# Rikorose/DeepFilterNet

Hardware: AMD Instinct MI355X
Metric: 48 kHz audio frames/sec (hop=480), DeepFilterNet3 enhance() (higher is better)
Workload: dtype f32 (storage and accumulation; GRU projections / recurrences, the fused DF-encoder convolutions and the pointwise halves of the ERB separable convolutions as fp16-split MFMAs: x = hi + lo in f16, hi*hi + hi*lo + lo*hi on v_mfma_f32_16x16x32_f16, ~2^-21 relative; see exact_fp32_ms_per_step); 1 GPU; DeepFilterNet3 (recalled shipped shape, conv_ch=64) enhance(pad=True), batch=256 clips x 10 s @48 kHz per GPU, 1002 STFT frames per clip; batch_per_gpu=256, global_batch=256, parallelism=clips sharded over 1 GPU(s); no collective, inputs_resident_in_hbm=True

## Files before the change

### deepfilternet_amd/csrc/dfx_nn_kernels.h

```cpp
#pragma once

#include "dfx_common.h"

#include <type_traits>

#define DFX_ACT_NONE 0
#define DFX_ACT_RELU 1
#define DFX_ACT_TANH 2
#define DFX_ACT_SIGMOID 3

static __device__ __forceinline__ float dfx_sigmoid(float x) { return 1.f / (1.f + expf(-x)); }
static __device__ __forceinline__ float dfx_act(float v, int act) {
    if (act == DFX_ACT_RELU) return fmaxf(v, 0.f);
    if (act == DFX_ACT_TANH) return tanhf(v);
    if (act == DFX_ACT_SIGMOID) return dfx_sigmoid(v);
    return v;
}

template <int I, int N, typename F>
static __device__ __forceinline__ void dfx_static_for(F &&f) {
    if constexpr (I < N) {
        f(std::integral_constant<int, I>{});
        dfx_static_for<I + 1, N>(f);
    }
// ... 267 lines not shown
                                         fmaxf(acc[nt][2] + biasr[nt].z, 0.f), fmaxf(acc[nt][3] + biasr[nt].w, 0.f));
        }
    }
}

static __device__ __forceinline__ void dfx_c0_patch(const float *__restrict__ feat, int64_t b, int64_t t, int f, bool valid,
                                                    int64_t T, int Fin, int L, int q, float (&bv)[5]) {
#pragma unroll
    for (int ks = 0; ks < 5; ++ks) {
        const int k = 4 * ks + q, tap = k >> 1, ch = k & 1, kt = tap / 3, kf = tap - 3 * kt;
        const int64_t tau = t - 2 + kt, tin = tau + L;
        const int fin = f - 1 + kf;
        float v = 0.f;
        if (valid && k < 18 && tau >= 0 && tin < T && fin >= 0 && fin < Fin) v = feat[((b * T + tin) * Fin + fin) * 2 + ch];
        bv[ks] = v;
    }
}

template <int C>
static __device__ __forceinline__ void dfx_c0_tile(const float (&areg0)[C / 16][5], const float4 (&bias0)[C / 16],
                                                   const float (&bv)[5], bool keep, float (&dst)[C / 4]) {
    constexpr int NT = C / 16;
    f32x4 acc[NT];
#pragma unroll
    for (int nt = 0; nt < NT; ++nt) acc[nt] = f32x4{0.f, 0.f, 0.f, 0.f};
#pragma unroll
    for (int ks = 0; ks < 5; ++ks)
#pragma unroll
        for (int nt = 0; nt < NT; ++nt) acc[nt] = __builtin_amdgcn_mfma_f32_16x16x4f32(areg0[nt][ks], bv[ks], acc[nt], 0, 0, 0);
#pragma unroll
    for (int nt = 0; nt < NT; ++nt) {
        dst[4 * nt + 0] = keep ? fmaxf(acc[nt][0] + bias0[nt].x, 0.f) : 0.f;
        dst[4 * nt + 1] = keep ? fmaxf(acc[nt][1] + bias0[nt].y, 0.f) : 0.f;
        dst[4 * nt + 2] = keep ? fmaxf(acc[nt][2] + bias0[nt].z, 0.f) : 0.f;
        dst[4 * nt + 3] = keep ? fmaxf(acc[nt][3] + bias0[nt].w, 0.f) : 0.f;
    }
}

struct DfxC01Args {
    const float *feat;
    const float *weff0;
    const float *bias0;
    const float *dw;
    const float *wt;
    const float *bias;
    float *out;
    int64_t B, T;
    int Fin, Fout, stride, L;
    int64_t t_begin;
    int64_t t_end;
};

template <int C>
__global__ void __launch_bounds__(DFX_PW_THREADS) dfx_k_df_conv01(DfxC01Args A) {
    constexpr int CPL = C / 4, NT = C / 16;
    __shared__ float4 dws[3 * C / 4];
    const int tid = threadIdx.x, lane = tid & 63, wave = tid >> 6, q = lane >> 4, jl = lane & 15;
    for (int i = tid; i < 3 * C / 4; i += DFX_PW_THREADS) dws[i] = reinterpret_cast<const float4 *>(A.dw)[i];
    float areg0[NT][5];
#pragma unroll
    for (int nt = 0; nt < NT; ++nt)
#pragma unroll
        for (int ks = 0; ks < 5; ++ks) areg0[nt][ks] = A.weff0[(4 * ks + q) * C + 16 * nt + jl];
    float areg[NT][CPL];
#pragma unroll
    for (int nt = 0; nt < NT; ++nt)
#pragma unroll
        for (int ks = 0; ks < CPL; ++ks) areg[nt][ks] = A.wt[(16 * (ks >> 2) + 4 * q + (ks & 3)) * C + 16 * nt + jl];
    float4 bias0[NT], biasr[NT];
#pragma unroll
    for (int nt = 0; nt < NT; ++nt) {
        bias0[nt] = reinterpret_cast<const float4 *>(A.bias0)[4 * nt + q];
        biasr[nt] = reinterpret_cast<const float4 *>(A.bias)[4 * nt + q];
    }
    __syncthreads();
    const int64_t Tn = A.t_end - A.t_begin;
    const int64_t total = A.B * Tn * A.Fout;
    const int64_t ntiles = (total + 15) / 16;
    for (int64_t tile = (int64_t)blockIdx.x * 4 + wave; tile < ntiles; tile += (int64_t)gridDim.x * 4) {
        const int64_t lpos = tile * 16 + jl;
        const bool valid = lpos < total;
        const int64_t rl = lpos / A.Fout;
        const int fo = (int)(lpos - rl * A.Fout);
        const int64_t b = rl / Tn, t = A.t_begin + (rl - b * Tn);
        const int64_t pos = (b * A.T + t) * A.Fout + fo;
        float u[CPL];
#pragma unroll
        for (int i = 0; i < CPL; ++i) u[i] = 0.f;
#pragma unroll
        for (int j = 0; j < 3; ++j) {
            const int fi = fo * A.stride + j - 1;
            const bool ok = valid && fi >= 0 && fi < A.Fin;
            float bv[5], c0v[CPL];
            dfx_c0_patch(A.feat, b, t, fi, ok, A.T, A.Fin, A.L, q, bv);
            dfx_c0_tile<C>(areg0, bias0, bv, ok, c0v);
#pragma unroll
            for (int nt = 0; nt < NT; ++nt) {
                const float4 w = dws[j * (C / 4) + 4 * nt + q];
                u[4 * nt + 0] += w.x * c0v[4 * nt + 0];
                u[4 * nt + 1] += w.y * c0v[4 * nt + 1];
                u[4 * nt + 2] += w.z * c0v[4 * nt + 2];
                u[4 * nt + 3] += w.w * c0v[4 * nt + 3];
            }
        }
        f32x4 acc[NT];
#pragma unroll
        for (int nt = 0; nt < NT; ++nt) acc[nt] = f32x4{0.f, 0.f, 0.f, 0.f};
#pragma unroll
        for (int ks = 0; ks < CPL; ++ks)
#pragma unroll
            for (int nt = 0; nt < NT; ++nt) acc[nt] = __builtin_amdgcn_mfma_f32_16x16x4f32(areg[nt][ks], u[ks], acc[nt], 0, 0, 0);
        if (valid) {
            float4 *op = reinterpret_cast<float4 *>(A.out + pos * C + 4 * q);
#pragma unroll
            for (int nt = 0; nt < NT; ++nt)
                op[4 * nt] = make_float4(fmaxf(acc[nt][0] + biasr[nt].x, 0.f), fmaxf(acc[nt][1] + biasr[nt].y, 0.f),
                                         fmaxf(acc[nt][2] + biasr[nt].z, 0.f), fmaxf(acc[nt][3] + biasr[nt].w, 0.f));
        }
    }
}

static __device__ __forceinline__ void dfx_c0_patch_load(const float *__restrict__ feat, int64_t b, int64_t t, int f, bool valid,
                                                         int64_t T, int Fin, int L, int q, float2 (&raw)[4], int64_t Ts = 0) {
    if (Ts <= 0) Ts = T;
#pragma unroll
    for (int i = 0; i < 4; ++i) {
        const int tap = 4 * q + i, kt = tap / 3, kf = tap - 3 * kt;
        const int64_t tau = t - 2 + kt, tin = tau + L;
        const int fin = f - 1 + kf;
        float2 v = make_float2(0.f, 0.f);
        if (valid && tap < 9 && tau >= 0 && tin < T && fin >= 0 && fin < Fin)
            v = *reinterpret_cast<const float2 *>(feat + ((b * Ts + tin) * Fin + fin) * 2);
        raw[i] = v;
    }
}

typedef unsigned dfx_words4 __attribute__((vector_size(16)));
struct DfxPatchPs {
    dfx_words4 h, l;
};
static __device__ __forceinline__ void dfx_c0_patch_ps(const DfxPatchPs &pk, dfx_h8 &ph, dfx_h8 &pl) {
    ph = __builtin_bit_cast(dfx_h8, pk.h);
    pl = __builtin_bit_cast(dfx_h8, pk.l);
}
static __device__ __forceinline__ void dfx_put_tap(float2 (&p)[4], int i, bool in, float2 v) { p[i] = make_float2(in ? v.x : 0.f, in ? v.y : 0.f); }
static __device__ __forceinline__ void dfx_put_tap(DfxPatchPs &p, int i, bool in, uint2 v) { p.h[i] = in ? v.x : 0u, p.l[i] = in ? v.y : 0u; }
static __device__ __forceinline__ void dfx_copy_patch(float2 (&d)[4], const float2 (&s)[4]) {
#pragma unroll
    for (int i = 0; i < 4; ++i) d[i] = s[i];
}
static __device__ __forceinline__ void dfx_copy_patch(DfxPatchPs &d, const DfxPatchPs &s) { d = s; }

template <int C>
static __device__ __forceinline__ void dfx_c0_tile_h3p(const dfx_h8 (&w0h)[C / 16], const dfx_h8 (&w0l)[C / 16],
                                                       const float4 (&bias0)[C / 16], float unscale0, const dfx_h8 ph, const dfx_h8 pl,
                                                       bool keep, float (&dst)[C / 4]) {
    constexpr int NT = C / 16;
    f32x4 acc[NT];
#pragma unroll
    for (int nt = 0; nt < NT; ++nt) acc[nt] = dfx_mfma_16x16x32_f16(w0l[nt], ph, f32x4{0.f, 0.f, 0.f, 0.f});
#pragma unroll
    for (int nt = 0; nt < NT; ++nt) acc[nt] = dfx_mfma_16x16x32_f16(w0h[nt], pl, acc[nt]);
#pragma unroll
    for (int nt = 0; nt < NT; ++nt) acc[nt] = dfx_mfma_16x16x32_f16(w0h[nt], ph, acc[nt]);
#pragma unroll
    for (int nt = 0; nt < NT; ++nt) {
        dst[4 * nt + 0] = keep ? fmaxf(acc[nt][0] * unscale0 + bias0[nt].x, 0.f) : 0.f;
        dst[4 * nt + 1] = keep ? fmaxf(acc[nt][1] * unscale0 + bias0[nt].y, 0.f) : 0.f;
        dst[4 * nt + 2] = keep ? fmaxf(acc[nt][2] * unscale0 + bias0[nt].z, 0.f) : 0.f;
        dst[4 * nt + 3] = keep ? fmaxf(acc[nt][3] * unscale0 + bias0[nt].w, 0.f) : 0.f;
    }
}
template <int C>
static __device__ __forceinline__ void dfx_c0_tile_h3(const dfx_h8 (&w0h)[C / 16], const dfx_h8 (&w0l)[C / 16],
                                                      const float4 (&bias0)[C / 16], float unscale0, const float2 (&raw)[4],
                                                      bool keep, float (&dst)[C / 4], float &amax) {
    float x[8];
#pragma unroll
    for (int i = 0; i < 4; ++i) x[2 * i] = raw[i].x, x[2 * i + 1] = raw[i].y;
    dfx_h8 ph, pl;
    dfx_split8_g(x, ph, pl, amax);
    dfx_c0_tile_h3p<C>(w0h, w0l, bias0, unscale0, ph, pl, keep, dst);
}
template <int C>
static __device__ __forceinline__ void dfx_c0_tile_h3(const dfx_h8 (&w0h)[C / 16], const dfx_h8 (&w0l)[C / 16],
                                                      const float4 (&bias0)[C / 16], float unscale0, const DfxPatchPs &raw,
                                                      bool keep, float (&dst)[C / 4], float &) {
    dfx_h8 ph, pl;
    dfx_c0_patch_ps(raw, ph, pl);
    dfx_c0_tile_h3p<C>(w0h, w0l, bias0, unscale0, ph, pl, keep, dst);
}

struct DfxC01hArgs {
    const float *feat;
    const dfx_h8 *w0f;
    const float *bias0;
    const float *dw;
    const dfx_h8 *wpf;
    const float *bias;
    float *out;
    int64_t B, T;
    int Fin, Fout, stride, L;
    float unscale0, unscale;
    int64_t t_begin;
    int64_t t_end;
    unsigned int *err;
    int64_t feat_T = 0;
};

template <int C>
#ifndef DFX_C01_MINB
#define DFX_C01_MINB 3
#endif
#ifndef DFX_C01_PIN
#define DFX_C01_PIN 0
#endif
#ifndef DFX_C01_EPI_BATCH
#define DFX_C01_EPI_BATCH 2
#endif
__global__ void __launch_bounds__(DFX_PW_THREADS, DFX_C01_MINB) dfx_k_df_conv01_h3(DfxC01hArgs A) {
    constexpr int CPL = C / 4, NT = C / 16, KC = C >= 32 ? C / 32 : 1, C4 = C / 4;
    static_assert(C % 32 == 0, "one k-chunk is 32 channels");
    __shared__ float4 dws[3 * C4];
    __shared__ float4 b0s[C4], b1s[C4];
    __shared__ dfx_h8 wps[NT * KC * 2 * 64];
    const int tid = threadIdx.x, lane = tid & 63, wave = tid >> 6, q = lane >> 4, jl = lane & 15;
    for (int i = tid; i < 3 * C4; i += DFX_PW_THREADS) dws[i] = reinterpret_cast<const float4 *>(A.dw)[i];
    for (int i = tid; i < C4; i += DFX_PW_THREADS) {
        b0s[i] = reinterpret_cast<const float4 *>(A.bias0)[i];
        b1s[i] = reinterpret_cast<const float4 *>(A.bias)[i];
    }
    for (int i = tid; i < NT * KC * 2 * 64; i += DFX_PW_THREADS) wps[i] = A.wpf[i];
    dfx_h8 w0h[NT], w0l[NT];
#pragma unroll
    for (int nt = 0; nt < NT; ++nt) {
        w0h[nt] = A.w0f[(nt * 2 + 0) * 64 + lane];
        w0l[nt] = A.w0f[(nt * 2 + 1) * 64 + lane];
    }
    __syncthreads();
    const unsigned Tn = (unsigned)(A.t_end - A.t_begin);
    const unsigned NF = (unsigned)A.B * Tn;
    const int TPF = (A.Fout + 15) >> 4;
    const unsigned nwaves = gridDim.x * 4;
    const int T32 = (int)A.T, Fin = A.Fin, Lk = A.L;
    int tdt[4], tdf[4];
    bool tok[4];
#pragma unroll
    for (int i = 0; i < 4; ++i) {
        const int tap = 4 * q + i, kt = tap / 3;
        tok[i] = tap < 9;
        tdt[i] = kt - 2 + Lk;
        tdf[i] = tap - 3 * kt - 1;
    }
    float2 raw[3][4];
    bool okj[3];
    const unsigned wid = (unsigned)blockIdx.x * 4 + (unsigned)dfx_wave_uniform(wave);
    const unsigned step_fr = nwaves / (unsigned)TPF;
    const int step_ft = (int)(nwaves - step_fr * (unsigned)TPF);
    unsigned nfr = wid / (unsigned)TPF;
    int nft = (int)(wid - nfr * (unsigned)TPF), nb = 0, nt_ = 0;
    bool nlive = nfr < NF;
    auto settle = [&]() {
        if (nlive) {
            nb = (int)(nfr / Tn);
            nt_ = (int)A.t_begin + (int)(nfr - (unsigned)nb * Tn);
        }
    };
    settle();
    auto issue = [&](int j) {
        const int fo = nft * 16 + jl;
        const int fi = fo * A.stride + j - 1;
        okj[j] = nlive && fo < A.Fout && fi >= 0 && fi < Fin;
        const float2 *clip = reinterpret_cast<const float2 *>(A.feat) + (int64_t)nb * (A.feat_T > 0 ? A.feat_T : (int64_t)T32) * Fin;
#pragma unroll
        for (int i = 0; i < 4; ++i) {
            const int tin = nt_ + tdt[i], fin = fi + tdf[i];
            float2 v = make_float2(0.f, 0.f);
            if (okj[j] && tok[i] && tin - Lk >= 0 && tin < T32 && fin >= 0 && fin < Fin) v = clip[tin * Fin + fin];
            raw[j][i] = v;
        }
    };
    float amax = 0.f;
#pragma unroll
    for (int j = 0; j < 3; ++j) issue(j);
    while (nlive) {
        const int fo_c = nft * 16 + jl;
        const bool valid = fo_c < A.Fout;
        const int64_t pos = ((int64_t)nb * T32 + nt_) * A.Fout + fo_c;
        nft += step_ft;
        nfr += step_fr;
        if (nft >= TPF) nft -= TPF, ++nfr;
        nlive = nfr < NF;
        settle();
        float u[CPL];
#pragma unroll
        for (int i = 0; i < CPL; ++i) u[i] = 0.f;
#pragma unroll
        for (int j = 0; j < 3; ++j) {
            float x[8];
#pragma unroll
            for (int i = 0; i < 4; ++i) x[2 * i] = raw[j][i].x, x[2 * i + 1] = raw[j][i].y;
            const bool keep = okj[j];
            dfx_h8 ph, pl;
            dfx_split8_g(x, ph, pl, amax);
            issue(j);
            f32x4 acc[NT];
#pragma unroll
            for (int nt = 0; nt < NT; ++nt) acc[nt] = dfx_mfma_16x16x32_f16(w0l[nt], ph, f32x4{0.f, 0.f, 0.f, 0.f});
#pragma unroll
            for (int nt = 0; nt < NT; ++nt) acc[nt] = dfx_mfma_16x16x32_f16(w0h[nt], pl, acc[nt]);
#pragma unroll
            for (int nt = 0; nt < NT; ++nt) acc[nt] = dfx_mfma_16x16x32_f16(w0h[nt], ph, acc[nt]);
#if DFX_C01_PIN
#pragma unroll
            for (int n0 = 0; n0 < NT; n0 += DFX_C01_EPI_BATCH) {
                float4 bz[DFX_C01_EPI_BATCH], w[DFX_C01_EPI_BATCH];
#pragma unroll
                for (int d = 0; d < DFX_C01_EPI_BATCH; ++d) {
                    bz[d] = b0s[4 * (n0 + d) + q], w[d] = dws[j * C4 + 4 * (n0 + d) + q];
                    DFX_OPAQUE(bz[d].x);
                    DFX_OPAQUE(bz[d].y);
                    DFX_OPAQUE(bz[d].z);
                    DFX_OPAQUE(bz[d].w);
                    DFX_OPAQUE(w[d].x);
// ... 160 lines not shown
                    const int tin = t + (tinfo[i] & 0xff) - 64, fin = fi + ((tinfo[i] >> 8) & 0xff) - 1;
                    float2 v = make_float2(0.f, 0.f);
                    if (ok && (tinfo[i] >> 16) && tin - Lk >= 0 && tin < T32 && fin >= 0 && fin < Fin) v = feat2[cbase + (unsigned)(tin * Fin + fin)];
                    dst[i] = v;
                }
            }
        };
        auto c0_tile = [&](auto jc, auto addc, auto nextc, int fo, Patch &rw, float (&u)[CPL], bool refill) {
            constexpr int j = decltype(jc)::value;
            constexpr bool ADD = decltype(addc)::value, NEXT = decltype(nextc)::value;
            const int fi = fo * A.stride + j - 1;
            const bool keep = live && fi >= 0 && fi < Fin;
            dfx_h8 ph, pl;
            if constexpr (PS) {
                dfx_c0_patch_ps(rw, ph, pl);
            } else {
                float x[8];
#pragma unroll
                for (int i = 0; i < 4; ++i) x[2 * i] = rw[i].x, x[2 * i + 1] = rw[i].y;
                dfx_split8_g(x, ph, pl, amax);
            }
            if (refill) issue_to(rw, j, fo + 1);
            int z0 = 0;
            DFX_OPAQUE(z0);
            dfx_h8 w0h[NT], w0l[NT];
#pragma unroll
            for (int nt = 0; nt < NT; ++nt) {
                w0h[nt] = w0s[(nt * 2 + 0) * 64 + lane + z0];
                w0l[nt] = w0s[(nt * 2 + 1) * 64 + lane + z0];
            }
            f32x4 acc[NT];
#pragma unroll
            for (int nt = 0; nt < NT; ++nt) acc[nt] = dfx_mfma_16x16x32_f16(w0l[nt], ph, f32x4{0.f, 0.f, 0.f, 0.f});
#pragma unroll
            for (int nt = 0; nt < NT; ++nt) acc[nt] = dfx_mfma_16x16x32_f16(w0h[nt], pl, acc[nt]);
#pragma unroll
            for (int nt = 0; nt < NT; ++nt) acc[nt] = dfx_mfma_16x16x32_f16(w0h[nt], ph, acc[nt]);
            auto epilogue = [&](auto allc) {
                constexpr bool ALL = decltype(allc)::value;
#pragma unroll
                for (int nt = 0; nt < NT; ++nt) {
                    const float4 bz = b0s[4 * nt + q];
                    const float v0 = ALL || keep ? fmaxf(acc[nt][0] * A.unscale0 + bz.x, 0.f) : 0.f, v1 = ALL || keep ? fmaxf(acc[nt][1] * A.unscale0 + bz.y, 0.f) : 0.f;
                    const float v2 = ALL || keep ? fmaxf(acc[nt][2] * A.unscale0 + bz.z, 0.f) : 0.f, v3 = ALL || keep ? fmaxf(acc[nt][3] * A.unscale0 + bz.w, 0.f) : 0.f;
                    if constexpr (ADD) {
                        const float4 w = dws[j * C4 + 4 * nt + q];
                        u[4 * nt + 0] += w.x * v0;
                        u[4 * nt + 1] += w.y * v1;
                        u[4 * nt + 2] += w.z * v2;
                        u[4 * nt + 3] += w.w * v3;
                    }
                    if constexpr (NEXT) {
                        const float4 wn = dws[4 * nt + q];
                        uns[nt * DFX_PW_THREADS + tid] = make_float4(0.f + wn.x * v0, 0.f + wn.y * v1, 0.f + wn.z * v2, 0.f + wn.w * v3);
                    }
                }
            };
            if constexpr (PS) {
                if (fi >= 0 && fi < Fin) epilogue(std::true_type{});
                else epilogue(std::false_type{});
            } else {
                epilogue(std::false_type{});
            }
        };
        using I0 = std::integral_constant<int, 0>;
        using I1 = std::integral_constant<int, 1>;
        using I2 = std::integral_constant<int, 2>;
        f32x4 accg = f32x4{0.f, 0.f, 0.f, 0.f};
        float ev[8];
        int ci = fo0 * KC;
        {
            float none[CPL];
            issue_to(raw[0], 0, fo0);
            c0_tile(I0{}, std::false_type{}, std::true_type{}, fo0, raw[0], none, false);
            issue_to(raw[0], 1, fo0);
            issue_to(raw[1], 2, fo0);
        }
        for (int fo = fo0; fo < fo1; ++fo) {
            float u[CPL];
#pragma unroll
            for (int nt = 0; nt < NT; ++nt) {
                const float4 c = uns[nt * DFX_PW_THREADS + tid];
                u[4 * nt + 0] = c.x, u[4 * nt + 1] = c.y, u[4 * nt + 2] = c.z, u[4 * nt + 3] = c.w;
            }
            c0_tile(I1{}, std::true_type{}, std::false_type{}, fo, raw[0], u, true);
            c0_tile(I2{}, std::true_type{}, std::true_type{}, fo, raw[1], u, true);
            dfx_h8 uh[KC], ul[KC];
#pragma unroll
            for (int kc = 0; kc < KC; ++kc) dfx_split8_g(u + 8 * kc, uh[kc], ul[kc], amax);
            int zoff = 0;
            DFX_OPAQUE(zoff);
            const dfx_h8 *wpl_ = wps + lane + zoff;
#pragma unroll
            for (int kc = 0; kc < KC; ++kc, ++ci) {
                int lz = lane;
                DFX_OPAQUE(lz);
                const dfx_h8 *wfl_ = A.wfc + lz;
                const dfx_h8 fh = wfl_[((size_t)ci * 2 + 0) * 64], fl = wfl_[((size_t)ci * 2 + 1) * 64];
                float c1v[8];
#pragma unroll
                for (int h = 0; h < 2; ++h) {
                    const int nt = 2 * kc + h;
                    f32x4 aa = f32x4{0.f, 0.f, 0.f, 0.f}, ab = aa, ac = aa;
#pragma unroll
                    for (int k2 = 0; k2 < KC; ++k2) {
                        const dfx_h8 wh = wpl_[((nt * KC + k2) * 2 + 0) * 64], wl = wpl_[((nt * KC + k2) * 2 + 1) * 64];
                        aa = dfx_mfma_16x16x32_f16(wl, uh[k2], aa);
                        ab = dfx_mfma_16x16x32_f16(wh, ul[k2], ab);
                        ac = dfx_mfma_16x16x32_f16(wh, uh[k2], ac);
                    }
                    const float4 bz = b1s[4 * nt + q];
                    c1v[4 * h + 0] = fmaxf(((aa[0] + ab[0]) + ac[0]) * A.unscale + bz.x, 0.f);
                    c1v[4 * h + 1] = fmaxf(((aa[1] + ab[1]) + ac[1]) * A.unscale + bz.y, 0.f);
                    c1v[4 * h + 2] = fmaxf(((aa[2] + ab[2]) + ac[2]) * A.unscale + bz.z, 0.f);
                    c1v[4 * h + 3] = fmaxf(((aa[3] + ab[3]) + ac[3]) * A.unscale + bz.w, 0.f);
                }
                dfx_h8 ch, cl;
                dfx_split8_g(c1v, ch, cl, amax);
                accg = dfx_mfma_16x16x32_f16(fl, ch, accg);
                accg = dfx_mfma_16x16x32_f16(fh, cl, accg);
                accg = dfx_mfma_16x16x32_f16(fh, ch, accg);
                if ((ci + 1) % A.cpg == 0) {
                    const int g = ci / A.cpg;
                    float4 e = make_float4(0.f, 0.f, 0.f, 0.f);
                    if (live) e = *reinterpret_cast<const float4 *>(A.e3 + (row * (unsigned)emb + (unsigned)(16 * g + 4 * q)));
                    const float4 v = make_float4(fmaxf(accg[0] * A.unscale_fc, 0.f) + e.x, fmaxf(accg[1] * A.unscale_fc, 0.f) + e.y,
                                                 fmaxf(accg[2] * A.unscale_fc, 0.f) + e.z, fmaxf(accg[3] * A.unscale_fc, 0.f) + e.w);
                    if (A.emb_in && live) *reinterpret_cast<float4 *>(A.emb_in + (row * (unsigned)emb + (unsigned)(16 * g + 4 * q))) = v;
                    accg = f32x4{0.f, 0.f, 0.f, 0.f};
                    if (g & 1) {
                        ev[4] = v.x, ev[5] = v.y, ev[6] = v.z, ev[7] = v.w;
                        const int jg = g >> 1;
                        const dfx_h8 *wil_ = A.win + lane + zoff;
                        const dfx_h8 ih = wil_[((size_t)jg * 2 + 0) * 64], il = wil_[((size_t)jg * 2 + 1) * 64];
                        dfx_h8 eh, el;
                        dfx_split8_g(ev, eh, el, amax);
                        f32x4 o = dfx_mfma_16x16x32_f16(il, eh, f32x4{0.f, 0.f, 0.f, 0.f});
                        o = dfx_mfma_16x16x32_f16(ih, el, o);
                        o = dfx_mfma_16x16x32_f16(ih, eh, o);
                        if (live)
                            *reinterpret_cast<float4 *>(A.xa + (row * (unsigned)(emb / 2) + (unsigned)(16 * jg + 4 * q))) =
                                make_float4(fmaxf(o[0] * A.unscale_in, 0.f), fmaxf(o[1] * A.unscale_in, 0.f), fmaxf(o[2] * A.unscale_in, 0.f),
                                            fmaxf(o[3] * A.unscale_in, 0.f));
                    } else {
                        ev[0] = v.x, ev[1] = v.y, ev[2] = v.z, ev[3] = v.w;
                    }
                }
            }
        }
    }
    if (amax >= DFX_H3_LIMIT && A.err) dfx_raise(A.err + 1);
}

struct DfxCphArgs {
    const float *feat;
    const dfx_h8 *w0f;
    const float *bias0;
    const dfx_h8 *wf;
    const float *bias;
    float *out;
    int64_t B, T;
    int Fd, NO, nfb, nseg, tseg, L;
    float unscale0, unscale;
    int64_t t_begin, t_zero, t_end;
    unsigned int *err;
    int64_t feat_T = 0;
    const int *t_zero_rows = nullptr;
    const uint2 *feat_ps = nullptr;
};

template <int C, int KT, bool PS = false>
__global__ void __launch_bounds__(256, 1) dfx_k_df_convp_h3(DfxCphArgs A) {
    using Patch = std::conditional_t<PS, DfxPatchPs, float2[4]>;
    using Elem = std::conditional_t<PS, uint2, float2>;
    constexpr int CPL = C / 4, NT = C / 16, KC = C >= 32 ? C / 32 : 1;
    static_assert(C % 32 == 0, "one k-chunk is 32 channels");
    const int tid = threadIdx.x, lane = tid & 63, wave = tid >> 6, q = lane >> 4, jl = lane & 15;
    float4 bias0[NT];
#pragma unroll
    for (int nt = 0; nt < NT; ++nt) bias0[nt] = reinterpret_cast<const float4 *>(A.bias0)[4 * nt + q];
    dfx_h8 w0h[NT], w0l[NT], wh[KT][KC], wl[KT][KC];
#pragma unroll
    for (int nt = 0; nt < NT; ++nt) {
        w0h[nt] = A.w0f[(nt * 2 + 0) * 64 + lane];
        w0l[nt] = A.w0f[(nt * 2 + 1) * 64 + lane];
    }
#pragma unroll
    for (int k = 0; k < KT; ++k)
#pragma unroll
        for (int kc = 0; kc < KC; ++kc) {
            wh[k][kc] = A.wf[((k * KC + kc) * 2 + 0) * 64 + lane];
            wl[k][kc] = A.wf[((k * KC + kc) * 2 + 1) * 64 + lane];
            DFX_PIN_AGPR(wh[k][kc]);
            DFX_PIN_AGPR(wl[k][kc]);
        }
    float biasr[4];
#pragma unroll
    for (int r = 0; r < 4; ++r) biasr[r] = A.bias[4 * q + r];
    const int64_t nruns = A.B * A.nfb * A.nseg;
    float amax = 0.f;
    const int Fd = A.Fd, T32 = (int)A.T, Lk = A.L;
    const int fT = (int)(A.feat_T > 0 ? A.feat_T : A.T);
    int toff[4], tdt[4], tdf[4];
#pragma unroll
    for (int i = 0; i < 4; ++i) {
        const int tap = 4 * q + i, kt = tap / 3;
        tdt[i] = tap < 9 ? kt - 2 + Lk : (1 << 20);
        tdf[i] = tap - 3 * kt - 1;
        toff[i] = (kt - 2 + Lk) * Fd + tdf[i];
    }
    const Elem *feat2;
    if constexpr (PS) feat2 = A.feat_ps;
    else feat2 = reinterpret_cast<const float2 *>(A.feat);
    for (int64_t run = (int64_t)blockIdx.x * 4 + dfx_wave_uniform(wave); run < nruns; run += (int64_t)gridDim.x * 4) {
        const int seg = (int)(run % A.nseg);
        const int64_t rest = run / A.nseg;
        const int fb = (int)(rest % A.nfb);
        const int64_t b = rest / A.nfb;
        const int f = fb * 16 + jl;
        const bool fvalid = f < Fd;
        const int64_t t0 = A.t_begin + (int64_t)seg * A.tseg;
        const int64_t t1 = (t0 + A.tseg < A.t_end) ? t0 + A.tseg : A.t_end;
        const unsigned cbase = (unsigned)b * (unsigned)fT * (unsigned)Fd;
        const int64_t tz = A.t_zero_rows ? (int64_t)A.t_zero_rows[b] : A.t_zero;
        auto patch = [&](int t, bool ok, Patch &rw) {
            const unsigned pbase = cbase + (unsigned)(t * Fd + f);
#pragma unroll
            for (int i = 0; i < 4; ++i) {
                const int tin = t + tdt[i], fin = f + tdf[i];
                const bool in = ok && tin - Lk >= 0 && tin < T32 && fin >= 0 && fin < Fd;
                dfx_put_tap(rw, i, in, feat2[in ? pbase + (unsigned)toff[i] : cbase]);
            }
        };
        dfx_h8 xh[KT][KC], xl[KT][KC];
        Patch raw;
        auto make_frame = [&](dfx_h8 (&dh)[KC], dfx_h8 (&dl)[KC], int64_t tau, const Patch &rw) {
            float c0v[CPL];
            dfx_c0_tile_h3<C>(w0h, w0l, bias0, A.unscale0, rw, fvalid && tau >= tz, c0v, amax);
#pragma unroll
            for (int kc = 0; kc < KC; ++kc) dfx_split8_g(c0v + 8 * kc, dh[kc], dl[kc], amax);
        };
        dfx_static_for<1, KT>([&](auto sc) {
            constexpr int sl = decltype(sc)::value;
            const int64_t tau = t0 - KT + sl;
            patch((int)tau, fvalid && tau >= 0, raw);
            make_frame(xh[sl], xl[sl], tau, raw);
        });
        patch((int)t0, fvalid, raw);
        for (int64_t tb = t0; tb < t1; tb += KT) {
            dfx_static_for<0, KT>([&](auto pc) {
                constexpr int ph = decltype(pc)::value;
                const int64_t t = tb + ph;
                if (t < t1) {
                    Patch cur;
                    dfx_copy_patch(cur, raw);
                    patch((int)t + 1, fvalid && t + 1 < t1, raw);
                    make_frame(xh[ph], xl[ph], t, cur);
                    f32x4 aa = f32x4{0.f, 0.f, 0.f, 0.f}, ab = aa, ac = aa;
                    dfx_static_for<0, KT>([&](auto kcn) {
                        constexpr int k = decltype(kcn)::value;
                        constexpr int sl = (ph + 1 + k) % KT;
#pragma unroll
                        for (int kc = 0; kc < KC; ++kc) {
                            const dfx_h8 whk = wh[k][kc], wlk = wl[k][kc];
                            aa = dfx_mfma_16x16x32_f16(wlk, xh[sl][kc], aa);
                            ab = dfx_mfma_16x16x32_f16(whk, xl[sl][kc], ab);
                            ac = dfx_mfma_16x16x32_f16(whk, xh[sl][kc], ac);
                        }
                    });
                    f32x4 acc;
#pragma unroll
                    for (int r = 0; r < 4; ++r) acc[r] = (aa[r] + ab[r]) + ac[r];
                    if (fvalid) {
                        float *op = A.out + ((b * (A.NO / 2) * A.T + t) * A.Fd + f) * 2;
#pragma unroll
                        for (int h = 0; h < 2; ++h)
                            if (4 * q + 2 * h < A.NO)
                                *reinterpret_cast<float2 *>(op + (int64_t)(2 * q + h) * A.T * A.Fd * 2) =
                                    make_float2(fmaxf(acc[2 * h] * A.unscale + biasr[2 * h], 0.f),
                                                fmaxf(acc[2 * h + 1] * A.unscale + biasr[2 * h + 1], 0.f));
                    }
                }
            });
        }
    }
    if (amax >= DFX_H3_LIMIT && A.err) dfx_raise(A.err + 1);
}

template <int C, int KT, bool REBUILD>
__global__ void __launch_bounds__(256, REBUILD ? 1 : 2) dfx_k_df_convp_step(DfxCphArgs A, f32x4 *pend, int slot_new, const unsigned char *par = nullptr,
                                                             const int *cnt = nullptr) {
    constexpr int CPL = C / 4, NT = C / 16, KC = C / 32, NS = KT - 1;
    static_assert(C % 32 == 0 && KT >= 2, "one k-chunk is 32 channels; kt = 1 has no history");
    const int tid = threadIdx.x, lane = tid & 63, wave = tid >> 6, q = lane >> 4, jl = lane & 15;
    dfx_h8 w0h[NT], w0l[NT];
    float4 bias0[NT];
#pragma unroll
    for (int nt = 0; nt < NT; ++nt) {
        w0h[nt] = A.w0f[(nt * 2 + 0) * 64 + lane];
        w0l[nt] = A.w0f[(nt * 2 + 1) * 64 + lane];
        bias0[nt] = reinterpret_cast<const float4 *>(A.bias0)[4 * nt + q];
    }
    float biasr[4];
#pragma unroll
    for (int r = 0; r < 4; ++r) biasr[r] = A.bias[4 * q + r];
    const int64_t nruns = A.B * A.nfb;
    const int64_t t = A.T - 1;
    float amax = 0.f;
    for (int64_t run = (int64_t)blockIdx.x * 4 + wave; run < nruns; run += (int64_t)gridDim.x * 4) {
        const int fb = (int)(run % A.nfb);
        const int64_t b = run / A.nfb;
        const int f = fb * 16 + jl;
        const bool fvalid = f < A.Fd;
        const int64_t tz = A.t_zero_rows ? (int64_t)A.t_zero_rows[dfx_wave_uniform((int)b)] : A.t_zero;
        const int half_in = par ? (int)(par[b] & 1) : 0, half_out = par ? half_in ^ 1 : 0, halves = par ? 2 : 1;
        const int slot0 = cnt ? cnt[b] % NS : slot_new;
        auto slot_ptr = [&](int j, int half) { return pend + ((((size_t)b * halves + half) * NS + (slot0 + j) % NS) * A.nfb + fb) * 64 + lane; };
        f32x4 sa[KT], sb[KT], sc[KT];
#pragma unroll
        for (int o = 0; o < KT; ++o) sa[o] = sb[o] = f32x4{0.f, 0.f, 0.f, 0.f}, sc[o] = f32x4{0.f, 0.f, 0.f, 0.f};
        if (!REBUILD) {
#pragma unroll
            for (int o = 0; o < NS; ++o) sc[o] = *slot_ptr(o, half_in);
        }
        dfx_static_for<(REBUILD ? 0 : KT - 1), KT>([&](auto dc) {
            constexpr int d = decltype(dc)::value;
            const int64_t tau = t - (KT - 1) + d;
            float2 raw[4];
            dfx_c0_patch_load(A.feat, b, tau, f, fvalid && tau >= 0, A.T, A.Fd, A.L, q, raw, A.feat_T);
            float c0v[CPL];
            dfx_c0_tile_h3<C>(w0h, w0l, bias0, A.unscale0, raw, fvalid && tau >= tz, c0v, amax);
            dfx_h8 xh[KC], xl[KC];
#pragma unroll
            for (int kc = 0; kc < KC; ++kc) dfx_split8_g(c0v + 8 * kc, xh[kc], xl[kc], amax);
            int zoff = 0;
            DFX_OPAQUE(zoff);
            const dfx_h8 *wfl = A.wf + lane + zoff;
#pragma unroll
            for (int kc = 0; kc < KC; ++kc) {
                dfx_h8 wl[KT], wh[KT];
                dfx_static_for<0, d + 1>([&](auto kcn) {
                    constexpr int k = decltype(kcn)::value;
                    wl[k] = wfl[((k * KC + kc) * 2 + 1) * 64], wh[k] = wfl[((k * KC + kc) * 2 + 0) * 64];
                });
                dfx_static_for<0, d + 1>([&](auto kcn) { constexpr int k = decltype(kcn)::value; sa[d - k] = dfx_mfma_16x16x32_f16(wl[k], xh[kc], sa[d - k]); });
                dfx_static_for<0, d + 1>([&](auto kcn) { constexpr int k = decltype(kcn)::value; sb[d - k] = dfx_mfma_16x16x32_f16(wh[k], xl[kc], sb[d - k]); });
                dfx_static_for<0, d + 1>([&](auto kcn) { constexpr int k = decltype(kcn)::value; sc[d - k] = dfx_mfma_16x16x32_f16(wh[k], xh[kc], sc[d - k]); });
            }
        });
        f32x4 sum[KT];
#pragma unroll
        for (int o = 0; o < KT; ++o)
#pragma unroll
            for (int r = 0; r < 4; ++r) sum[o][r] = (sa[o][r] + sb[o][r]) + sc[o][r];
#pragma unroll
        for (int o = 1; o < KT; ++o) *slot_ptr(o, half_out) = sum[o];
        if (fvalid) {
            float *op = A.out + ((b * (A.NO / 2) * A.T + t) * A.Fd + f) * 2;
#pragma unroll
            for (int h = 0; h < 2; ++h)
                if (4 * q + 2 * h < A.NO)
                    *reinterpret_cast<float2 *>(op + (int64_t)(2 * q + h) * A.T * A.Fd * 2) =
                        make_float2(fmaxf(sum[0][2 * h] * A.unscale + biasr[2 * h], 0.f), fmaxf(sum[0][2 * h + 1] * A.unscale + biasr[2 * h + 1], 0.f));
        }
    }
    if (amax >= DFX_H3_LIMIT && A.err) dfx_raise(A.err + 1);
}

#define DFX_CH_NF 2
template <int C, int MODE, typename Epi>
static __device__ __forceinline__ void dfx_chain_stage(const float *in, int Fin, int Fout, int stride, int npos,
                                                       const float4 *dws, const float (&areg)[C / 16][C / 4],
                                                       const float4 (&biasr)[C / 16], int lane, Epi &&epi) {
    constexpr int CPL = C / 4, NT = C / 16, V4 = CPL / 4, LD = C + 4;
    const int q = lane >> 4, jl = lane & 15;
    for (int p0 = 0; p0 < npos; p0 += 16) {
        const int p = p0 + jl;
        const bool valid = p < npos;
        const int fr = p / Fout, fo = p - fr * Fout;
        float u[CPL];
#pragma unroll
        for (int i = 0; i < CPL; ++i) u[i] = 0.f;
#pragma unroll
        for (int j = 0; j < 3; ++j) {
            int fi;
            bool ok;
            if (MODE == DFX_PW_MODE_DW3) {
                fi = fo * stride + j - 1;
                ok = fi >= 0 && fi < Fin;
            } else {
                const int num = fo + 1 - j;
                fi = num >> 1;
                ok = num >= 0 && (num & 1) == 0 && fi < Fin;
            }
            if (valid && ok) {
                const float4 *xp = reinterpret_cast<const float4 *>(in + (fr * Fin + fi) * LD + CPL * q);
#pragma unroll
                for (int v = 0; v < V4; ++v) {
                    const float4 xv = xp[v];
                    const float4 w = dws[j * (C / 4) + V4 * q + v];
                    u[4 * v + 0] += w.x * xv.x;
                    u[4 * v + 1] += w.y * xv.y;
                    u[4 * v + 2] += w.z * xv.z;
                    u[4 * v + 3] += w.w * xv.w;
                }
            }
        }
        f32x4 acc[NT];
#pragma unroll
        for (int nt = 0; nt < NT; ++nt) acc[nt] = f32x4{0.f, 0.f, 0.f, 0.f};
#pragma unroll
        for (int ks = 0; ks < CPL; ++ks)
#pragma unroll
            for (int nt = 0; nt < NT; ++nt) acc[nt] = __builtin_amdgcn_mfma_f32_16x16x4f32(areg[nt][ks], u[ks], acc[nt], 0, 0, 0);
#pragma unroll
        for (int nt = 0; nt < NT; ++nt)
            epi(p, valid, nt,
                make_float4(fmaxf(acc[nt][0] + biasr[nt].x, 0.f), fmaxf(acc[nt][1] + biasr[nt].y, 0.f),
                            fmaxf(acc[nt][2] + biasr[nt].z, 0.f), fmaxf(acc[nt][3] + biasr[nt].w, 0.f)));
    }
}

template <int C>
static __device__ __forceinline__ void dfx_chain_load_w(const float *wt, const float *bias, int lane, float (&areg)[C / 16][C / 4],
                                                        float4 (&biasr)[C / 16]) {
    constexpr int CPL = C / 4, NT = C / 16;
    const int q = lane >> 4, jl = lane & 15;
#pragma unroll
    for (int nt = 0; nt < NT; ++nt) {
#pragma unroll
        for (int ks = 0; ks < CPL; ++ks) areg[nt][ks] = wt[(CPL * q + ks) * C + 16 * nt + jl];
        biasr[nt] = reinterpret_cast<const float4 *>(bias)[4 * nt + q];
    }
}

template <int C>
static __device__ __forceinline__ void dfx_chain_load_w_h3(const dfx_h8 *frags, const float *bias, int lane, dfx_h8 (&ahi)[C / 16][C / 32],
                                                           dfx_h8 (&alo)[C / 16][C / 32], float4 (&biasr)[C / 16]) {
// ... 3258 lines not shown
```

Before: 24.28 million frames/s.

## Software-pipeline DF conv kernel: prefetch two frames ahead, delay stores, interleave MFMA/VALU

```diff
diff --git a/deepfilternet_amd/csrc/dfx_nn_kernels.h b/deepfilternet_amd/csrc/dfx_nn_kernels.h
--- a/deepfilternet_amd/csrc/dfx_nn_kernels.h
+++ b/deepfilternet_amd/csrc/dfx_nn_kernels.h
@@ -443,24 +443,37 @@
 static __device__ __forceinline__ void dfx_copy_patch(DfxPatchPs &d, const DfxPatchPs &s) { d = s; }
 
 template <int C>
+static __device__ __forceinline__ void dfx_c0_tile_h3_products(const dfx_h8 (&w0h)[C / 16], const dfx_h8 (&w0l)[C / 16], const dfx_h8 ph,
+                                                               const dfx_h8 pl, f32x4 (&acc)[C / 16]) {
+    constexpr int NT = C / 16;
+#pragma unroll
+    for (int nt = 0; nt < NT; ++nt) acc[nt] = dfx_mfma_16x16x32_f16(w0l[nt], ph, f32x4{0.f, 0.f, 0.f, 0.f});
+#pragma unroll
+    for (int nt = 0; nt < NT; ++nt) acc[nt] = dfx_mfma_16x16x32_f16(w0h[nt], pl, acc[nt]);
+#pragma unroll
+    for (int nt = 0; nt < NT; ++nt) acc[nt] = dfx_mfma_16x16x32_f16(w0h[nt], ph, acc[nt]);
+}
+template <int C>
+static __device__ __forceinline__ void dfx_c0_tile_h3_epilogue(const f32x4 (&acc)[C / 16], const float4 (&bias0)[C / 16], float unscale0, bool keep,
+                                                               float (&dst)[C / 4]) {
+    constexpr int NT = C / 16;
+#pragma unroll
+    for (int nt = 0; nt < NT; ++nt) {
+        const float v0 = fmaxf(acc[nt][0] * unscale0 + bias0[nt].x, 0.f), v1 = fmaxf(acc[nt][1] * unscale0 + bias0[nt].y, 0.f);
+        const float v2 = fmaxf(acc[nt][2] * unscale0 + bias0[nt].z, 0.f), v3 = fmaxf(acc[nt][3] * unscale0 + bias0[nt].w, 0.f);
+        dst[4 * nt + 0] = keep ? v0 : 0.f;
+        dst[4 * nt + 1] = keep ? v1 : 0.f;
+        dst[4 * nt + 2] = keep ? v2 : 0.f;
+        dst[4 * nt + 3] = keep ? v3 : 0.f;
+    }
+}
+template <int C>
 static __device__ __forceinline__ void dfx_c0_tile_h3p(const dfx_h8 (&w0h)[C / 16], const dfx_h8 (&w0l)[C / 16],
                                                        const float4 (&bias0)[C / 16], float unscale0, const dfx_h8 ph, const dfx_h8 pl,
                                                        bool keep, float (&dst)[C / 4]) {
-    constexpr int NT = C / 16;
-    f32x4 acc[NT];
-#pragma unroll
-    for (int nt = 0; nt < NT; ++nt) acc[nt] = dfx_mfma_16x16x32_f16(w0l[nt], ph, f32x4{0.f, 0.f, 0.f, 0.f});
-#pragma unroll
-    for (int nt = 0; nt < NT; ++nt) acc[nt] = dfx_mfma_16x16x32_f16(w0h[nt], pl, acc[nt]);
-#pragma unroll
-    for (int nt = 0; nt < NT; ++nt) acc[nt] = dfx_mfma_16x16x32_f16(w0h[nt], ph, acc[nt]);
-#pragma unroll
-    for (int nt = 0; nt < NT; ++nt) {
-        dst[4 * nt + 0] = keep ? fmaxf(acc[nt][0] * unscale0 + bias0[nt].x, 0.f) : 0.f;
-        dst[4 * nt + 1] = keep ? fmaxf(acc[nt][1] * unscale0 + bias0[nt].y, 0.f) : 0.f;
-        dst[4 * nt + 2] = keep ? fmaxf(acc[nt][2] * unscale0 + bias0[nt].z, 0.f) : 0.f;
-        dst[4 * nt + 3] = keep ? fmaxf(acc[nt][3] * unscale0 + bias0[nt].w, 0.f) : 0.f;
-    }
+    f32x4 acc[C / 16];
+    dfx_c0_tile_h3_products<C>(w0h, w0l, ph, pl, acc);
+    dfx_c0_tile_h3_epilogue<C>(acc, bias0, unscale0, keep, dst);
 }
 template <int C>
 static __device__ __forceinline__ void dfx_c0_tile_h3(const dfx_h8 (&w0h)[C / 16], const dfx_h8 (&w0l)[C / 16],
@@ -927,6 +940,40 @@
     if (amax >= DFX_H3_LIMIT && A.err) dfx_raise(A.err + 1);
 }
 
+#ifndef DFX_CPH_ABLATE
+#define DFX_CPH_ABLATE 0
+#endif
+#ifndef DFX_CPH_TRACE
+#define DFX_CPH_TRACE 0
+#endif
+#ifndef DFX_CPH_PARENT_LOOP
+#define DFX_CPH_PARENT_LOOP 0
+#endif
+#ifndef DFX_CPH_VALU_C0
+#define DFX_CPH_VALU_C0 4
+#endif
+#ifndef DFX_CPH_VALU_TAPS
+#define DFX_CPH_VALU_TAPS 5
+#endif
+template <int N, int V>
+static __device__ __forceinline__ void dfx_sched_mfma_valu() {
+#pragma unroll
+    for (int i = 0; i < N; ++i) {
+        DFX_SCHED_GROUP(0x008, 1);
+        DFX_SCHED_GROUP(0x002, V);
+    }
+}
+#if DFX_CPH_TRACE
+#define DFX_CPH_TICK(i)                                                               \
+    do {                                                                                \
+        unsigned long long now_;                                                        \
+        asm volatile("s_memtime %0\n\ts_waitcnt lgkmcnt(0)" : "=s"(now_)::"memory");    \
+        tk[i] += now_ - tlast;                                                          \
+        tlast = now_;                                                                   \
+    } while (0)
+#else
+#define DFX_CPH_TICK(i) do { } while (0)
+#endif
 struct DfxCphArgs {
     const float *feat;
     const dfx_h8 *w0f;
@@ -942,7 +989,29 @@
     int64_t feat_T = 0;
     const int *t_zero_rows = nullptr;
     const uint2 *feat_ps = nullptr;
+#if DFX_CPH_TRACE
+    unsigned long long *trace = nullptr;
+#endif
 };
+static __device__ __forceinline__ void dfx_patch_ready(float2 (&p)[4]) {
+#pragma unroll
+    for (int i = 0; i < 4; ++i) {
+        DFX_OPAQUE(p[i].x);
+        DFX_OPAQUE(p[i].y);
+    }
+}
+static __device__ __forceinline__ void dfx_patch_ready(DfxPatchPs &p) {
+    DFX_OPAQUE(p.h);
+    DFX_OPAQUE(p.l);
+}
+template <typename E>
+static __device__ __forceinline__ void dfx_loads_ready(E (&ld)[4]) {
+#pragma unroll
+    for (int i = 0; i < 4; ++i) {
+        DFX_OPAQUE(ld[i].x);
+        DFX_OPAQUE(ld[i].y);
+    }
+}
 
 template <int C, int KT, bool PS = false>
 __global__ void __launch_bounds__(256, 1) dfx_k_df_convp_h3(DfxCphArgs A) {
@@ -974,6 +1043,9 @@
     for (int r = 0; r < 4; ++r) biasr[r] = A.bias[4 * q + r];
     const int64_t nruns = A.B * A.nfb * A.nseg;
     float amax = 0.f;
+#if DFX_CPH_TRACE
+    unsigned long long tk[4] = {0, 0, 0, 0}, tlast, nframes = 0;
+#endif
     const int Fd = A.Fd, T32 = (int)A.T, Lk = A.L;
     const int fT = (int)(A.feat_T > 0 ? A.feat_T : A.T);
     int toff[4], tdt[4], tdf[4];
@@ -1004,14 +1076,50 @@
             for (int i = 0; i < 4; ++i) {
                 const int tin = t + tdt[i], fin = f + tdf[i];
                 const bool in = ok && tin - Lk >= 0 && tin < T32 && fin >= 0 && fin < Fd;
-                dfx_put_tap(rw, i, in, feat2[in ? pbase + (unsigned)toff[i] : cbase]);
+                if constexpr (DFX_CPH_ABLATE & 2) dfx_put_tap(rw, i, false, Elem{});
+                else dfx_put_tap(rw, i, in, feat2[in ? pbase + (unsigned)toff[i] : cbase]);
+            }
+        };
+        auto patch_in = [&](int t, bool ok, int i) {
+            return ok & (t + tdt[i] - Lk >= 0) & (t + tdt[i] < T32) & (f + tdf[i] >= 0) & (f + tdf[i] < Fd);
+        };
+        auto patch_load = [&](int t, bool ok, Elem (&ld)[4]) {
+            const unsigned pbase = cbase + (unsigned)(t * Fd + f);
+#pragma unroll
+            for (int i = 0; i < 4; ++i) {
+                if constexpr (DFX_CPH_ABLATE & 2) ld[i] = Elem{};
+                else {
+                    const bool in = patch_in(t, ok, i);
+                    ld[i] = feat2[in ? pbase + (unsigned)toff[i] : cbase];
+                }
+            }
+        };
+        auto patch_select = [&](int t, bool ok, const Elem (&ld)[4], Patch &rw) {
+#pragma unroll
+            for (int i = 0; i < 4; ++i) dfx_put_tap(rw, i, patch_in(t, ok, i), ld[i]);
+        };
+        const bool st_on = !(DFX_CPH_ABLATE & 1) || A.NO < 0;
+        auto store_out = [&](int64_t t, const float2 (&v)[2]) {
+            if (fvalid && st_on) {
+                float *op = A.out + ((b * (A.NO / 2) * A.T + t) * A.Fd + f) * 2;
+#pragma unroll
+                for (int h = 0; h < 2; ++h)
+                    if (4 * q + 2 * h < A.NO) *reinterpret_cast<float2 *>(op + (int64_t)(2 * q + h) * A.T * A.Fd * 2) = v[h];
             }
         };
         dfx_h8 xh[KT][KC], xl[KT][KC];
         Patch raw;
         auto make_frame = [&](dfx_h8 (&dh)[KC], dfx_h8 (&dl)[KC], int64_t tau, const Patch &rw) {
             float c0v[CPL];
-            dfx_c0_tile_h3<C>(w0h, w0l, bias0, A.unscale0, rw, fvalid && tau >= tz, c0v, amax);
+            if constexpr (PS && !DFX_CPH_PARENT_LOOP) {
+                dfx_h8 p_h, p_l;
+                dfx_c0_patch_ps(rw, p_h, p_l);
+                f32x4 acc0[NT];
+                dfx_c0_tile_h3_products<C>(w0h, w0l, p_h, p_l, acc0);
+                DFX_MFMA_GUARD();
+                dfx_c0_tile_h3_epilogue<C>(acc0, bias0, A.unscale0, fvalid && tau >= tz, c0v);
+            } else
+                dfx_c0_tile_h3<C>(w0h, w0l, bias0, A.unscale0, rw, fvalid && tau >= tz, c0v, amax);
 #pragma unroll
             for (int kc = 0; kc < KC; ++kc) dfx_split8_g(c0v + 8 * kc, dh[kc], dl[kc], amax);
         };
@@ -1021,44 +1129,128 @@
             patch((int)tau, fvalid && tau >= 0, raw);
             make_frame(xh[sl], xl[sl], tau, raw);
         });
-        patch((int)t0, fvalid, raw);
-        for (int64_t tb = t0; tb < t1; tb += KT) {
-            dfx_static_for<0, KT>([&](auto pc) {
-                constexpr int ph = decltype(pc)::value;
-                const int64_t t = tb + ph;
-                if (t < t1) {
-                    Patch cur;
-                    dfx_copy_patch(cur, raw);
-                    patch((int)t + 1, fvalid && t + 1 < t1, raw);
-                    make_frame(xh[ph], xl[ph], t, cur);
-                    f32x4 aa = f32x4{0.f, 0.f, 0.f, 0.f}, ab = aa, ac = aa;
-                    dfx_static_for<0, KT>([&](auto kcn) {
-                        constexpr int k = decltype(kcn)::value;
-                        constexpr int sl = (ph + 1 + k) % KT;
-#pragma unroll
-                        for (int kc = 0; kc < KC; ++kc) {
-                            const dfx_h8 whk = wh[k][kc], wlk = wl[k][kc];
-                            aa = dfx_mfma_16x16x32_f16(wlk, xh[sl][kc], aa);
-                            ab = dfx_mfma_16x16x32_f16(whk, xl[sl][kc], ab);
-                            ac = dfx_mfma_16x16x32_f16(whk, xh[sl][kc], ac);
+#if DFX_CPH_TRACE
+        asm volatile("s_memtime %0\n\ts_waitcnt lgkmcnt(0)" : "=s"(tlast)::"memory");
+        nframes += (unsigned long long)(t1 - t0);
+#endif
+        if constexpr (PS && !DFX_CPH_PARENT_LOOP) {
+            float2 held[2] = {make_float2(0.f, 0.f), make_float2(0.f, 0.f)};
+            constexpr int U = (KT % 2) ? 2 * KT : KT;
+            Elem ld2[2][4];
+            patch_load((int)t0, fvalid, ld2[0]);
+            patch_load((int)t0 + 1, fvalid && t0 + 1 < t1, ld2[1]);
+            for (int64_t tb = t0; tb < t1; tb += U) {
+                bool whole = false;
+                auto frame = [&](auto &self, auto pc) {
+                    constexpr int ph = decltype(pc)::value % KT;
+                    Elem(&ld)[4] = ld2[decltype(pc)::value & 1];
+                    const int64_t t = tb + decltype(pc)::value;
+                    if (t < t1) {
+                        dfx_loads_ready(ld);
+                        DFX_CPH_TICK(0);
+                        DFX_SCHED_BARRIER();
+                        if (t > t0) store_out(t - 1, held);
+                        DFX_CPH_TICK(3);
+                        DFX_SCHED_BARRIER();
+                        Patch cur;
+                        patch_select((int)t, fvalid, ld, cur);
+                        patch_load((int)t + 2, fvalid && t + 2 < t1, ld);
+                        dfx_h8 p_h, p_l;
+                        dfx_c0_patch_ps(cur, p_h, p_l);
+                        f32x4 acc0[NT];
+                        dfx_c0_tile_h3_products<C>(w0h, w0l, p_h, p_l, acc0);
+                        dfx_sched_mfma_valu<3 * NT, DFX_CPH_VALU_C0>();
+                        DFX_SCHED_BARRIER();
+                        f32x4 aa = f32x4{0.f, 0.f, 0.f, 0.f}, ab = aa, ac = aa;
+                        auto tap = [&](auto kcn) {
+                            constexpr int k = decltype(kcn)::value;
+                            constexpr int sl = (ph + 1 + k) % KT;
+#pragma unroll
+                            for (int kc = 0; kc < KC; ++kc) {
+                                const dfx_h8 whk = wh[k][kc], wlk = wl[k][kc];
+                                aa = dfx_mfma_16x16x32_f16(wlk, xh[sl][kc], aa);
+                                ab = dfx_mfma_16x16x32_f16(whk, xl[sl][kc], ab);
+                                ac = dfx_mfma_16x16x32_f16(whk, xh[sl][kc], ac);
+                            }
+                        };
+                        dfx_static_for<0, KT - 1>(tap);
+                        float c0v[CPL];
+                        dfx_c0_tile_h3_epilogue<C>(acc0, bias0, A.unscale0, fvalid && t >= tz, c0v);
+#pragma unroll
+                        for (int kc = 0; kc < KC; ++kc) dfx_split8_g(c0v + 8 * kc, xh[ph][kc], xl[ph][kc], amax);
+                        dfx_sched_mfma_valu<3 * KC * (KT - 1), DFX_CPH_VALU_TAPS>();
+                        DFX_SCHED_BARRIER();
+                        tap(std::integral_constant<int, KT - 1>{});
+                        f32x4 acc;
+#pragma unroll
+                        for (int r = 0; r < 4; ++r) acc[r] = (aa[r] + ab[r]) + ac[r];
+#pragma unroll
+                        for (int h = 0; h < 2; ++h)
+                            held[h] = make_float2(fmaxf(acc[2 * h] * A.unscale + biasr[2 * h], 0.f),
+                                                  fmaxf(acc[2 * h + 1] * A.unscale + biasr[2 * h + 1], 0.f));
+                        DFX_CPH_TICK(1);
+                        DFX_SCHED_BARRIER();
+                        if constexpr (decltype(pc)::value + 1 < U) self(self, std::integral_constant<int, decltype(pc)::value + 1>{});
+                        else whole = true;
+                    }
+                };
+                frame(frame, std::integral_constant<int, 0>{});
+                if (!whole) break;
+            }
+            if (t1 > t0) store_out(t1 - 1, held);
+        } else {
+            patch((int)t0, fvalid, raw);
+            for (int64_t tb = t0; tb < t1; tb += KT) {
+                dfx_static_for<0, KT>([&](auto pc) {
+                    constexpr int ph = decltype(pc)::value;
+                    const int64_t t = tb + ph;
+                    if (t < t1) {
+                        Patch cur;
+                        dfx_copy_patch(cur, raw);
+#if DFX_CPH_TRACE
+                        dfx_patch_ready(cur);
+                        DFX_CPH_TICK(0);
+#endif
+                        patch((int)t + 1, fvalid && t + 1 < t1, raw);
+                        make_frame(xh[ph], xl[ph], t, cur);
+                        DFX_CPH_TICK(1);
+                        f32x4 aa = f32x4{0.f, 0.f, 0.f, 0.f}, ab = aa, ac = aa;
+                        dfx_static_for<0, KT>([&](auto kcn) {
+                            constexpr int k = decltype(kcn)::value;
+                            constexpr int sl = (ph + 1 + k) % KT;
+#pragma unroll
+                            for (int kc = 0; kc < KC; ++kc) {
+                                const dfx_h8 whk = wh[k][kc], wlk = wl[k][kc];
+                                aa = dfx_mfma_16x16x32_f16(wlk, xh[sl][kc], aa);
+                                ab = dfx_mfma_16x16x32_f16(whk, xl[sl][kc], ab);
+                                ac = dfx_mfma_16x16x32_f16(whk, xh[sl][kc], ac);
+                            }
+                        });
+                        f32x4 acc;
+#pragma unroll
+                        for (int r = 0; r < 4; ++r) acc[r] = (aa[r] + ab[r]) + ac[r];
+                        DFX_CPH_TICK(2);
+                        if (fvalid && st_on) {
+                            float *op = A.out + ((b * (A.NO / 2) * A.T + t) * A.Fd + f) * 2;
+#pragma unroll
+                            for (int h = 0; h < 2; ++h)
+                                if (4 * q + 2 * h < A.NO)
+                                    *reinterpret_cast<float2 *>(op + (int64_t)(2 * q + h) * A.T * A.Fd * 2) =
+                                        make_float2(fmaxf(acc[2 * h] * A.unscale + biasr[2 * h], 0.f),
+                                                    fmaxf(acc[2 * h + 1] * A.unscale + biasr[2 * h + 1], 0.f));
                         }
-                    });
-                    f32x4 acc;
-#pragma unroll
-                    for (int r = 0; r < 4; ++r) acc[r] = (aa[r] + ab[r]) + ac[r];
-                    if (fvalid) {
-                        float *op = A.out + ((b * (A.NO / 2) * A.T + t) * A.Fd + f) * 2;
-#pragma unroll
-                        for (int h = 0; h < 2; ++h)
-                            if (4 * q + 2 * h < A.NO)
-                                *reinterpret_cast<float2 *>(op + (int64_t)(2 * q + h) * A.T * A.Fd * 2) =
-                                    make_float2(fmaxf(acc[2 * h] * A.unscale + biasr[2 * h], 0.f),
-                                                fmaxf(acc[2 * h + 1] * A.unscale + biasr[2 * h + 1], 0.f));
+                        DFX_CPH_TICK(3);
                     }
-                }
-            });
-        }
-    }
+                });
+            }
+        }
+    }
+#if DFX_CPH_TRACE
+    if (tid == 0 && A.trace) {
+        for (int i = 0; i < 4; ++i) A.trace[(size_t)blockIdx.x * 5 + i] = tk[i];
+        A.trace[(size_t)blockIdx.x * 5 + 4] = nframes;
+    }
+#endif
     if (amax >= DFX_H3_LIMIT && A.err) dfx_raise(A.err + 1);
 }
 
```

After: 24.79 million frames/s (median of 6 runs). 1.02x the previous value.
